# MingXiangL/AttentionShift

Hardware: AMD Instinct MI355X
Metric: images/sec (1024^2, ViT-B) hot path: backbone attention fwd + attention-shift pseudo-labels (higher is better)
Workload: dtype bf16

## Files before the change

attentionshift_amd/_lib.py:

```python
import ctypes
import os

_HERE = os.path.dirname(os.path.abspath(__file__))
LIB_PATH = os.path.join(_HERE, "libattnshift_hip.so")

AS_F32, AS_BF16 = 0, 1

_c_void_p, _c_int, _c_float, _c_size_t = ctypes.c_void_p, ctypes.c_int, ctypes.c_float, ctypes.c_size_t
_c_double = ctypes.c_double

SIGNATURES = {
    "as_version": (_c_int, []),
    "as_last_error": (ctypes.c_char_p, []),
    "as_npad": (_c_int, [_c_int]),
    "as_linear_fwd": (_c_int, [_c_void_p] * 4 + [_c_int] * 5 + [_c_void_p]),
    "as_linear_small_fwd": (_c_int, [_c_void_p, _c_int, _c_void_p, _c_void_p, _c_void_p] + [_c_int] * 5 + [_c_void_p]),
    "as_linear_sk_workspace_bytes": (_c_size_t, [_c_int] * 3),
    "as_linear_sk_fwd": (_c_int, [_c_void_p] * 4 + [_c_int] * 5 + [_c_void_p, _c_size_t, _c_void_p]),
    "as_linear_gelu_fwd": (_c_int, [_c_void_p] * 5 + [_c_int] * 4 + [_c_void_p]),
    "as_linear_dgelu_fwd": (_c_int, [_c_void_p] * 4 + [_c_int] * 4 + [_c_void_p]),
    "as_deconv2x2_fwd": (_c_int, [_c_void_p] * 4 + [_c_int] * 6 + [_c_void_p]),
    "as_qkv_fwd": (_c_int, [_c_void_p] * 6 + [_c_int] * 5 + [_c_void_p]),
    "as_sdpa_fwd_workspace_bytes": (_c_size_t, [_c_int] * 4),
    "as_sdpa_fwd": (_c_int, [_c_void_p] * 6 + [_c_size_t] + [_c_int] * 4 + [_c_void_p]),
# ... 13 lines not shown
    "as_linear_bwd_workspace_bytes": (ctypes.c_size_t, [_c_int] * 3),
    "as_linear_bwd": (_c_int, [_c_void_p] * 6 + [_c_int] * 5 + [_c_void_p, ctypes.c_size_t, _c_void_p]),
    "as_linear_bwd_dgelu": (_c_int, [_c_void_p] * 7 + [_c_int] * 5 + [_c_void_p, ctypes.c_size_t, _c_void_p]),
    "as_assemble_tokens": (_c_int, [_c_void_p] * 3 + [_c_int] * 5 + [_c_void_p]),
    "as_maxpool_nhwc": (_c_int, [_c_void_p] * 2 + [_c_int] * 5 + [ctypes.c_longlong, _c_void_p]),
    "as_mask_count": (_c_int, [_c_void_p] * 2 + [_c_int] * 2 + [_c_void_p]),
    "as_window_attn_bwd_workspace_bytes": (_c_size_t, [_c_int] * 5),
    "as_window_attn_bwd": (_c_int, [_c_void_p] * 8 + [_c_size_t] + [_c_int] * 8 + [_c_void_p]),
    "as_attn_fwd": (_c_int, [_c_void_p] * 12 + [_c_size_t] + [_c_int] * 5 + [_c_void_p]),
    "as_attn_mean_rows": (_c_int, [_c_void_p] * 4 + [_c_int] * 6 + [_c_void_p]),
    "as_rollout_rfrag_bytes": (_c_size_t, [_c_int] * 3),
    "as_rollout_pack": (_c_int, [_c_void_p] * 2 + [_c_int] * 4 + [_c_void_p]),
    "as_rollout_top": (_c_int, [_c_void_p] * 5 + [_c_int] * 5 + [_c_void_p]),
    "as_rollout_step_workspace_bytes": (_c_size_t, [_c_int] * 3),
    "as_rollout_step": (_c_int, [_c_void_p] * 8 + [_c_size_t] + [_c_int] * 5 + [_c_void_p]),
    "as_ccl_2d": (_c_int, [_c_void_p] * 2 + [_c_int] * 3 + [_c_void_p]),
    "as_cam_boxes_workspace_bytes": (_c_size_t, [_c_int] * 4),
    "as_cam_boxes": (_c_int, [_c_void_p] * 2 + [_c_float] * 2 + [_c_int] * 4 + [_c_void_p] * 5 + [_c_size_t, _c_void_p]),
    "as_cam_sample_masks_workspace_bytes": (_c_size_t, [_c_int] * 4),
    "as_cam_sample_masks": (_c_int, [_c_void_p] * 3 + [_c_int] * 4 + [_c_float] * 2 + [_c_void_p] * 3 + [_c_size_t, _c_void_p]),
    "as_mask_candidates_workspace_bytes": (_c_size_t, [_c_int] * 3),
    "as_mask_candidates": (_c_int, [_c_void_p] * 3 + [_c_float] * 3 + [_c_int] + [_c_void_p] * 5 + [_c_size_t]
                           + [_c_int] * 3 + [_c_void_p]),
    "as_part_select": (_c_int, [_c_void_p] * 7 + [_c_int] * 5 + [_c_void_p] * 8 + [_c_void_p]),
    "as_part_stats": (_c_int, [_c_void_p] * 3 + [_c_float] + [_c_void_p] * 4 + [_c_int] * 3 + [_c_void_p]),
    "as_filter_parts": (_c_int, [_c_void_p] * 2 + [_c_float] * 2 + [_c_void_p] + [_c_int] * 3 + [_c_void_p]),
    "as_draw_distinct": (_c_int, [_c_void_p, _c_int, _c_int] + [_c_void_p] * 5 + [_c_int] * 3 + [_c_void_p]),
    "as_mt_sample_ranks": (_c_int, [_c_void_p] * 4 + [_c_int] * 2 + [_c_void_p]),
    "as_mt_perm_ranks": (_c_int, [_c_void_p] * 4 + [_c_int] * 2 + [_c_void_p]),
    "as_small_attn_fwd": (_c_int, [_c_void_p] * 3 + [_c_int] * 5 + [_c_void_p]),
# ... 66 lines not shown
```

attentionshift_amd/csrc/rollout.hip:

```cpp
#include <stdlib.h>
#include "common.h"

namespace {

constexpr int HD = 64, RO_NT = 256;
constexpr float LOG2E = 1.44269504088896340736f;

template <typename T> struct KjCfg { static constexpr int PITCH = HD * (int)sizeof(T) + 16; };

__device__ __forceinline__ size_t rf_slot(int b, int nkb, int i, int k) {
  const int rem = k & 31, s2 = rem >> 4, r16 = rem & 15;
  const int lane = (i & 31) + 32 * ((r16 & 7) >> 2), t = (r16 >> 3) * 4 + (r16 & 3);
  return ((((((size_t)b * nkb + (k >> 5)) * 4 + (i >> 5)) * 2 + s2) * 64) + lane) * 8 + t;
}
__device__ __forceinline__ size_t rf_frag(int b, int nkb, int kb, int ib, int s2, int lane) {
  return ((((((size_t)b * nkb + kb) * 4 + ib) * 2 + s2) * 64) + lane) * 8;
}

template <typename T>
__device__ __forceinline__ f32x16 pbar_tile(const T* __restrict__ q, const T* __restrict__ k,
                                            const float* __restrict__ lse, const char* kj_lds, int b, int h,
                                            int N, int Npad, int i0, int j0, int li, int half) {
  f32x16 pbar;
#pragma unroll
  for (int r = 0; r < 16; ++r) pbar[r] = 0.0f;
  const int irow = min(i0 + li, N - 1);
  const int jrow = min(j0 + li, N - 1);
  for (int hh = 0; hh < h; ++hh) {
    const size_t bh = (size_t)b * h + hh;
    f32x16 s;
#pragma unroll
    for (int r = 0; r < 16; ++r) s[r] = 0.0f;
#pragma unroll
    for (int ks = 0; ks < 4; ++ks) {
      Frag<T> fa, fb;
      fa.load16B(q + qf_frag(bh, Npad, irow, ks, half));
      if (kj_lds != nullptr)
        fb.load16B(reinterpret_cast<const T*>(kj_lds + ((size_t)hh * 32 + li) * KjCfg<T>::PITCH) + ks * 16 + half * 8);
      else
        fb.load16B(k + (bh * Npad + jrow) * HD + ks * 16 + half * 8);
      s = mma32(fa, fb, s);
    }
    const float* lrow = lse + bh * N;
#pragma unroll
    for (int r = 0; r < 16; ++r) {
      const int row = min(i0 + acc_row(r, half), N - 1);
      pbar[r] += __builtin_amdgcn_exp2f(s[r] - lrow[row] * LOG2E);
    }
  }
  const float inv_h = 1.0f / (float)h;
#pragma unroll
  for (int r = 0; r < 16; ++r) pbar[r] *= inv_h;
  return pbar;
}

template <typename T, bool TOP>
__global__ __launch_bounds__(RO_NT) void attn_mean_rows_kernel(const T* __restrict__ q, const T* __restrict__ k,
                                                               const float* __restrict__ lse,
                                                               float* __restrict__ out, T* __restrict__ rf_out, int B,
                                                               int N, int Npad, int h, int row0, int nrows) {
  const int lane = threadIdx.x & 63, wave = threadIdx.x >> 6;
  const int li = lane & 31, half = lane >> 5;
  const int jb = blockIdx.x * 4 + wave, ib = blockIdx.y, b = blockIdx.z;
  const int j0 = jb * 32, i0 = ib * 32;
  if (j0 >= N) return;
  const f32x16 p = pbar_tile<T>(q, k, lse, nullptr, b, h, N, Npad, row0 + i0, j0, li, half);
  const int j = j0 + li;
  const int nkb = (N + 31) / 32;
#pragma unroll
  for (int r = 0; r < 16; ++r) {
    const int i = i0 + acc_row(r, half);
    float v = p[r];
    if (TOP) v = 0.5f * (v + ((row0 + i) == j ? 1.0f : 0.0f));
    const bool live = i < nrows && j < N;
    if (live) out[((size_t)b * nrows + i) * N + j] = v;
    if (rf_out != nullptr && i < 128) rf_out[rf_slot(b, nkb, i, j)] = from_f32<T>(live ? v : 0.0f);
  }
}

template <typename T> struct Kj2 {
  static constexpr int PITCH = sizeof(T) == 2 ? 128 : (HD * 4 + 16);
  __device__ static __forceinline__ int off(int row, int elem) {
    if (sizeof(T) == 2) return row * 128 + ((((elem >> 3) ^ (row & 7))) << 4);
    return row * PITCH + elem * 4;
  }
};

template <typename T, int HPW>
__global__ __launch_bounds__(RO_NT) void rollout_step2_kernel(const T* __restrict__ q, const T* __restrict__ k,
                                                              const float* __restrict__ lse,
                                                              const float* __restrict__ Rin, const T* __restrict__ rf_in,
                                                              float* __restrict__ Rout, T* __restrict__ rf_out,
                                                              float* __restrict__ part, int B, int N, int Npad, int h,
                                                              int Trows, int nsplit, int xbufs) {
  extern __shared__ __attribute__((aligned(16))) char smem[];
  constexpr bool PREFETCH = sizeof(T) == 2;
  const int tid = threadIdx.x, lane = tid & 63, wave = tid >> 6;
  const int li = lane & 31, half = lane >> 5;
  const int j0 = blockIdx.x * 32, b = blockIdx.y, split = blockIdx.z;
  char* kj = smem;
  float4* xchg = reinterpret_cast<float4*>(smem + (size_t)h * 32 * Kj2<T>::PITCH);

  {
    constexpr int CPR = HD * (int)sizeof(T) / 16;
    const int total = h * 32 * CPR;
    for (int c = tid; c < total; c += RO_NT) {
      const int hh = c / (32 * CPR), rem = c % (32 * CPR);
      const int jr = rem / CPR, ch = rem % CPR;
      const int jrow = min(j0 + jr, N - 1);
// ... 97 lines not shown
    if (xbufs == 1) __syncthreads();
  }

  if (own_rows) {
    const int j = j0 + li;
#pragma unroll
    for (int r = 0; r < 16; ++r) {
      const int i = wave * 32 + acc_row(r, half);
      const bool live = i < Trows && j < N;
      if (nsplit > 1) {
        if (live) part[(((size_t)split * B + b) * Trows + i) * N + j] = acc[r];
        continue;
      }
      float v = 0.0f;
      if (live) {
        const size_t idx = ((size_t)b * Trows + i) * N + j;
        v = 0.5f * (acc[r] + Rin[idx]);
        Rout[idx] = v;
      }
      if (rf_out != nullptr) rf_out[rf_slot(b, nkb, i, j)] = from_f32<T>(v);
    }
  }
}

#ifndef AS_ROLLOUT_ABLATE
#define AS_ROLLOUT_ABLATE 0
#endif
template <typename T> __device__ __forceinline__ f32x16 inject_rows(float x, int half);
template <> __device__ __forceinline__ f32x16 inject_rows<float>(float x, int half) {
  f32x16 z;
#pragma unroll
// ... 10 lines not shown
  const __bf16 mid = (__bf16)r1;
  const __bf16 lo = (__bf16)(r1 - (float)mid);
  const __bf16 zero = (__bf16)0.0f, one = (__bf16)1.0f;
  Frag<__bf16> fa, fb;
  fa.v = bf16x8{hi, mid, lo, zero, zero, zero, zero, zero};
  fb.v = bf16x8{one, one, one, zero, zero, zero, zero, zero};
  return mma32(fa, fb, z);
}

template <typename T>
__global__ __launch_bounds__(RO_NT, 3) void rollout_step3_kernel(const T* __restrict__ q, const T* __restrict__ k,
                                                                 const float* __restrict__ lse,
                                                                 const float* __restrict__ Rin, const T* __restrict__ rf_in,
                                                                 float* __restrict__ Rout, T* __restrict__ rf_out,
                                                                 float* __restrict__ part, int B, int N, int Npad, int h,
                                                                 int Trows, int nsplit) {
  extern __shared__ __attribute__((aligned(16))) char smem[];
  const int tid = threadIdx.x, lane = tid & 63, wave = tid >> 6;
  const int li = lane & 31, half = lane >> 5;
  const int j0 = blockIdx.x * 32, b = blockIdx.y, split = blockIdx.z;
  char* kj = smem;
  {
    constexpr int CPR = HD * (int)sizeof(T) / 16;
    const int total = h * 32 * CPR;
    for (int c = tid; c < total; c += RO_NT) {
      const int hh = c / (32 * CPR), rem = c % (32 * CPR);
      const int jr = rem / CPR, ch = rem % CPR;
      const int jrow = min(j0 + jr, N - 1);
      const uint4 u = *reinterpret_cast<const uint4*>(
          reinterpret_cast<const char*>(k + (((size_t)b * h + hh) * Npad + jrow) * HD) + ch * 16);
      const int elem = ch * (16 / (int)sizeof(T));
// ... 92 lines not shown
                   red[((2 * 2 + x) * 16 + r) * 64 + lane]) + red[((3 * 2 + x) * 16 + r) * 64 + lane];
    }
  }
  if (wave * 32 < Trows) {
    const int j = j0 + li;
#pragma unroll
    for (int r = 0; r < 16; ++r) {
      const int i = wave * 32 + acc_row(r, half);
      const bool live = i < Trows && j < N;
      if (nsplit > 1) {
        if (live) part[(((size_t)split * B + b) * Trows + i) * N + j] = mine[r];
        continue;
      }
      float v = 0.0f;
      if (live) {
        const size_t idx = ((size_t)b * Trows + i) * N + j;
        v = 0.5f * (mine[r] + Rin[idx]);
        Rout[idx] = v;
      }
      if (rf_out != nullptr) rf_out[rf_slot(b, nkb, i, j)] = from_f32<T>(v);
    }
  }
}

constexpr int R4_HPG = 4;
constexpr int R4_QBYTES = R4_HPG * 4 * 1024;
constexpr int R4_LSE = R4_QBYTES + 8 * 1024;
constexpr int R4_STAGE = R4_LSE + 1024;
#ifndef AS_R4_OCC1
#define AS_R4_OCC1 3
#endif
template <int NIB> struct R4Cfg { static constexpr int NSTAGE = NIB == 1 ? 2 : 3, OCC = NIB == 1 ? AS_R4_OCC1 : 2; };

typedef __attribute__((ext_vector_type(4))) unsigned r4_u32x4;
template <int OFF> __device__ __forceinline__ void r4_lds_read128(r4_u32x4& dst, unsigned addr) {
  asm volatile("ds_read_b128 %0, %1 offset:%2" : "=v"(dst) : "v"(addr), "n"(OFF));
}
__device__ __forceinline__ void r4_lds_read128_dyn(r4_u32x4& dst, unsigned addr) {
  asm volatile("ds_read_b128 %0, %1" : "=v"(dst) : "v"(addr));
}
__device__ __forceinline__ void r4_wait_lds(r4_u32x4& a, r4_u32x4& b, r4_u32x4& c, r4_u32x4& d) {
  asm volatile("s_waitcnt lgkmcnt(0)" : "+v"(a), "+v"(b), "+v"(c), "+v"(d));
  __builtin_amdgcn_sched_barrier(0);
}
__device__ __forceinline__ void r4_wait_lds8(r4_u32x4& a, r4_u32x4& b, r4_u32x4& c, r4_u32x4& d, r4_u32x4& e, r4_u32x4& f,
                                             r4_u32x4& g, r4_u32x4& h) {
  asm volatile("s_waitcnt lgkmcnt(0)" : "+v"(a), "+v"(b), "+v"(c), "+v"(d), "+v"(e), "+v"(f), "+v"(g), "+v"(h));
// ... 10 lines not shown
__device__ __forceinline__ void r4_dma16(unsigned voff, const char* sbase, unsigned dst) {
  unsigned keep;
  asm volatile("s_mov_b32 %0, m0\n\ts_mov_b32 m0, %3\n\ts_nop 0\n\tglobal_load_lds_dwordx4 %1, %2\n\ts_mov_b32 m0, %0"
               : "=&s"(keep) : "v"(voff), "s"(sbase), "s"(dst) : "memory");
}
__device__ __forceinline__ void r4_dma4(unsigned voff, const char* sbase, unsigned dst) {
  unsigned keep;
  asm volatile("s_mov_b32 %0, m0\n\ts_mov_b32 m0, %3\n\ts_nop 0\n\tglobal_load_lds_dword %1, %2\n\ts_mov_b32 m0, %0"
               : "=&s"(keep) : "v"(voff), "s"(sbase), "s"(dst) : "memory");
}

template <int NIB>
__global__ __launch_bounds__(RO_NT, R4Cfg<NIB>::OCC) void rollout_step4_kernel(const __bf16* __restrict__ q, const __bf16* __restrict__ k,
                                                                 const float* __restrict__ lse, const __bf16* __restrict__ rf_in,
                                                                 float* __restrict__ part, int B, int N, int Npad, int h,
                                                                 int Trows, int ksplit) {
  extern __shared__ __attribute__((aligned(16))) char smem[];
  constexpr int R4_NSTAGE = R4Cfg<NIB>::NSTAGE;
  const int tid = threadIdx.x, lane = tid & 63, wave = __builtin_amdgcn_readfirstlane(tid >> 6);
  const int li = lane & 31, half = lane >> 5;
  const int ngroups = h / R4_HPG;
  const int j0 = blockIdx.x * 128 + wave * 32, b = blockIdx.y;
  const int hg = blockIdx.z % ngroups, split = blockIdx.z / ngroups;
  const int nkb = (N + 31) / 32;
  const int nib = min((Trows + 31) / 32, NIB);
  const int kb0 = (int)((long long)nkb * split / ksplit), kb1 = (int)((long long)nkb * (split + 1) / ksplit);
  const int nblk = kb1 - kb0;
  const size_t bh0 = (size_t)b * h + hg * R4_HPG;

  Frag<__bf16> fk[R4_HPG][4];
  {
// ... 28 lines not shown
#pragma unroll
    for (int r = 0; r < 16; ++r) acc[ib][r] = 0.0f;
  const float inv_h = 1.0f / (float)h;
  const unsigned lbase = (unsigned)(size_t)(const __attribute__((address_space(3))) char*)smem + lane * 16;

  if (nblk > 0) stage(kb0, 0);
  if (R4_NSTAGE > 2 && nblk > 1) stage(kb0 + 1, 1);

  for (int it = 0; it < nblk; ++it) {
    const int kb = kb0 + it, buf = it % R4_NSTAGE;
    if (AS_ROLLOUT_ABLATE != 11) {
      if (R4_NSTAGE == 2 || it + 1 >= nblk) asm volatile("s_waitcnt vmcnt(0)" ::: "memory");
      else if (NIB == 4 || wave == 0) asm volatile("s_waitcnt vmcnt(7)" ::: "memory");
      else asm volatile("s_waitcnt vmcnt(5)" ::: "memory");
    }
    {
      float own;
      const unsigned a_own = (unsigned)(size_t)(const __attribute__((address_space(3))) char*)smem + buf * R4_STAGE + R4_LSE + wave * 256 + lane * 4;
      asm volatile("ds_read_b32 %0, %1\n\ts_waitcnt lgkmcnt(0)" : "=v"(own) : "v"(a_own) : "memory");
      own *= -LOG2E;
      asm volatile("ds_write_b32 %0, %1\n\ts_waitcnt lgkmcnt(0)" :: "v"(a_own), "v"(own) : "memory");
    }
    if (AS_ROLLOUT_ABLATE != 14) __builtin_amdgcn_s_barrier();
    if (AS_ROLLOUT_ABLATE != 11 && it + R4_NSTAGE - 1 < nblk) stage(kb + R4_NSTAGE - 1, (it + R4_NSTAGE - 1) % R4_NSTAGE);
    const unsigned sb = lbase + buf * R4_STAGE;
    const unsigned cb = (unsigned)(size_t)(const __attribute__((address_space(3))) char*)smem + buf * R4_STAGE + R4_LSE + half * 16;
    r4_u32x4 fc[2][4];
    auto read_c = [&](int hh, r4_u32x4 (&c)[4]) {
      const unsigned a = cb + hh * 256;
      r4_lds_read128_dyn(c[0], a);
      r4_lds_read128<32>(c[1], a);
// ... 79 lines not shown
    __builtin_amdgcn_sched_barrier(0);
#pragma unroll
    for (int s2 = 0; s2 < 2; ++s2)
#pragma unroll
      for (int ib = 0; ib < NIB; ++ib)
        if (ib < nib) {
          Frag<__bf16> f;
          f.v = *reinterpret_cast<bf16x8*>(&fr[ib][s2]);
          if (AS_ROLLOUT_ABLATE != 15) acc[ib] = mma32(f, fp[s2], acc[ib]);
          else acc[ib][0] += (float)f.v[0] + (float)fp[s2].v[0];
        }
  }

  const int pidx = split * ngroups + hg;
  const int j = j0 + li;
  if (j < N) {
#pragma unroll
    for (int ib = 0; ib < NIB; ++ib)
#pragma unroll
      for (int r = 0; r < 16; ++r) {
        const int i = ib * 32 + acc_row(r, half);
        if (i < Trows) part[(((size_t)pidx * B + b) * Trows + i) * N + j] = acc[ib][r] * inv_h;
      }
  }
}

bool rollout_force_v3() {
  static const bool v = getenv("AS_ROLLOUT_V3") != nullptr;
  return v;
}

constexpr int R4_MAXPARTS = 16;
int rollout4_ksplit(int B, int N, int h, int slots) {
  static const int forced = [] { const char* e = getenv("AS_R4_KS"); return e ? atoi(e) : 0; }();
  if (forced > 0 && forced * (h / R4_HPG) <= 16) return forced;
  const int units = as_ceil_div(N, 128) * B * (h / R4_HPG);
  int best = 1;
  float best_eff = 0.0f;
  for (int ks = 1; ks * (h / R4_HPG) <= R4_MAXPARTS && ks <= 8; ++ks) {
    const int wgs = units * ks;
    const float eff = (float)wgs / (float)(as_ceil_div(wgs, slots) * slots);
    if (eff > best_eff + 0.02f) { best_eff = eff; best = ks; }
  }
  return best;
}

template <typename T>
__global__ __launch_bounds__(64) void rollout_finish_kernel(const float* __restrict__ part, const float* __restrict__ Rin,
                                                            float* __restrict__ Rout, T* __restrict__ rf_out, int B, int N,
                                                            int Trows, int nsplit) {
  const int nkb = (N + 31) / 32;
  const int j = blockIdx.x * 64 + threadIdx.x, i = blockIdx.y, b = blockIdx.z;
  if (j >= nkb * 32) return;
  float v = 0.0f;
  if (i < Trows && j < N) {
    const size_t idx = ((size_t)b * Trows + i) * N + j;
    float a = 0.0f;
    for (int sp = 0; sp < nsplit; ++sp) a += part[(size_t)sp * B * Trows * N + idx];
    v = 0.5f * (a + Rin[idx]);
    Rout[idx] = v;
  }
  if (rf_out != nullptr) rf_out[rf_slot(b, nkb, i, j)] = from_f32<T>(v);
}

template <typename T>
int launch_rollout_step2(const void* q, const void* k, const float* lse, const float* Rin, const void* rf_in, float* Rout,
                         void* rf_out, float* part, int nsplit, int B, int N, int h, int Trows, hipStream_t s) {
  const int Npad = as_round_up(N, 64);
  const int hpw = as_ceil_div(h, 4);
  dim3 grid(as_ceil_div(N, 32), B, nsplit);
  const size_t kbytes = (size_t)h * 32 * Kj2<T>::PITCH, slab = 4 * 4 * 64 * sizeof(float4);
  const int xbufs = kbytes + 2 * slab <= 160 * 1024 ? 2 : 1;
  const size_t lds = kbytes + xbufs * slab;
  AS_REQUIRE(lds <= 160 * 1024, AS_E_UNSUPPORTED, "rollout_step: LDS %zu B exceeds 160 KiB (h=%d)", lds, h);
#define AS_RO2(HPW)                                                                                            \
  do {                                                                                                         \
    (void)hipFuncSetAttribute((const void*)rollout_step2_kernel<T, HPW>, hipFuncAttributeMaxDynamicSharedMemorySize, \
                              (int)lds);                                                                       \
    hipLaunchKernelGGL((rollout_step2_kernel<T, HPW>), grid, dim3(RO_NT), lds, s, (const T*)q, (const T*)k, lse, Rin, \
                       (const T*)rf_in, Rout, (T*)rf_out, part, B, N, Npad, h, Trows, nsplit, xbufs);          \
  } while (0)
  if (sizeof(T) == 2 && h % R4_HPG == 0 && part != nullptr && nsplit == R4_MAXPARTS && !rollout_force_v3()) {
    const int ng = h / R4_HPG;
    const int ks = rollout4_ksplit(B, N, h, 512);
    const size_t lds4 = (size_t)(Trows <= 32 ? R4Cfg<1>::NSTAGE : R4Cfg<4>::NSTAGE) * R4_STAGE;
    if (Trows <= 32) {
      (void)hipFuncSetAttribute((const void*)rollout_step4_kernel<1>, hipFuncAttributeMaxDynamicSharedMemorySize, (int)lds4);
      hipLaunchKernelGGL(rollout_step4_kernel<1>, dim3(as_ceil_div(N, 128), B, ks * ng), dim3(RO_NT), lds4, s, (const __bf16*)q,
                         (const __bf16*)k, lse, (const __bf16*)rf_in, part, B, N, Npad, h, Trows, ks);
    } else {
      (void)hipFuncSetAttribute((const void*)rollout_step4_kernel<4>, hipFuncAttributeMaxDynamicSharedMemorySize, (int)lds4);
      hipLaunchKernelGGL(rollout_step4_kernel<4>, dim3(as_ceil_div(N, 128), B, ks * ng), dim3(RO_NT), lds4, s, (const __bf16*)q,
                         (const __bf16*)k, lse, (const __bf16*)rf_in, part, B, N, Npad, h, Trows, ks);
    }
    AS_CHECK_LAUNCH("rollout_step4");
    dim3 fg(as_ceil_div(as_ceil_div(N, 32) * 32, 64), as_round_up(Trows, 32), B);
    hipLaunchKernelGGL((rollout_finish_kernel<T>), fg, dim3(64), 0, s, (const float*)part, Rin, Rout, (T*)rf_out, B, N,
                       Trows, ks * ng);
    AS_CHECK_LAUNCH("rollout_finish");
    return AS_OK;
  }
  if (sizeof(T) == 2 && h >= 8 && (getenv("AS_ROLLOUT_V2") == nullptr)) {
    const size_t lds3 = (size_t)h * 32 * Kj2<T>::PITCH;
    (void)hipFuncSetAttribute((const void*)rollout_step3_kernel<T>, hipFuncAttributeMaxDynamicSharedMemorySize, (int)lds3);
    hipLaunchKernelGGL((rollout_step3_kernel<T>), grid, dim3(RO_NT), lds3, s, (const T*)q, (const T*)k, lse, Rin,
                       (const T*)rf_in, Rout, (T*)rf_out, part, B, N, Npad, h, Trows, nsplit);
  } else {
  switch (hpw) {
    case 1: AS_RO2(1); break;
    case 2: AS_RO2(2); break;
    case 3: AS_RO2(3); break;
    case 4: AS_RO2(4); break;
    default: AS_REQUIRE(false, AS_E_UNSUPPORTED, "rollout_step: h=%d heads (max 16)", h);
  }
  }
#undef AS_RO2
  AS_CHECK_LAUNCH("rollout_step2");
  if (nsplit > 1) {
    dim3 fg(as_ceil_div(as_ceil_div(N, 32) * 32, 64), as_round_up(Trows, 32), B);
    hipLaunchKernelGGL((rollout_finish_kernel<T>), fg, dim3(64), 0, s, (const float*)part, Rin, Rout, (T*)rf_out, B, N,
                       Trows, nsplit);
    AS_CHECK_LAUNCH("rollout_finish");
  }
  return AS_OK;
}

int rollout_nsplit(int B, int N) {
  const int wgs = as_ceil_div(N, 32) * B;
  int ns = 1;
  while (ns < 16 && wgs * ns < 2048) ns *= 2;
  return wgs >= 2048 ? 1 : ns;
}

template <typename T>
int launch_mean_rows(const void* q, const void* k, const float* lse, float* out, void* rf_out, int B, int N, int h,
                     int row0, int nrows, bool top, hipStream_t s) {
  const int Npad = as_round_up(N, 64);
  dim3 grid(as_ceil_div(as_ceil_div(N, 32), 4), as_ceil_div(nrows, 32), B);
  if (top)
    hipLaunchKernelGGL((attn_mean_rows_kernel<T, true>), grid, dim3(RO_NT), 0, s, (const T*)q, (const T*)k, lse,
                       out, (T*)rf_out, B, N, Npad, h, row0, nrows);
  else
    hipLaunchKernelGGL((attn_mean_rows_kernel<T, false>), grid, dim3(RO_NT), 0, s, (const T*)q, (const T*)k, lse,
                       out, (T*)rf_out, B, N, Npad, h, row0, nrows);
  AS_CHECK_LAUNCH("attn_mean_rows");
  return AS_OK;
}

}

extern "C" size_t as_rollout_rfrag_bytes(int B, int N, int dtype) {
  if (B <= 0 || N <= 0) return 0;
  return (size_t)B * as_ceil_div(N, 32) * 4 * 2 * 64 * 8 * (dtype == AS_BF16 ? 2 : 4);
}

extern "C" int as_attn_mean_rows(const void* q, const void* k, const float* lse, float* out, int B, int N, int h,
                                 int row0, int nrows, int dtype, as_stream_t stream) {
  AS_REQUIRE(q && k && lse && out, AS_E_BADARG, "as_attn_mean_rows: null pointer");
  AS_REQUIRE(B > 0 && N > 0 && h > 0 && row0 >= 0 && nrows > 0 && row0 + nrows <= N, AS_E_BADARG,
// ... 27 lines not shown

extern "C" int as_rollout_pack(const float* R, void* rf, int B, int N, int T, int dtype, as_stream_t stream) {
  AS_REQUIRE(R && rf, AS_E_BADARG, "as_rollout_pack: null pointer");
  AS_REQUIRE(B > 0 && N > 0 && T > 0 && T <= 128, AS_E_BADARG, "as_rollout_pack: bad sizes N=%d T=%d", N, T);
  dim3 grid(as_ceil_div(as_ceil_div(N, 32) * 32, 64), as_round_up(T, 32), B);
  if (dtype == AS_BF16)
    hipLaunchKernelGGL(rollout_pack_kernel<__bf16>, grid, dim3(64), 0, (hipStream_t)stream, R, (__bf16*)rf, B, N, T);
  else if (dtype == AS_F32)
    hipLaunchKernelGGL(rollout_pack_kernel<float>, grid, dim3(64), 0, (hipStream_t)stream, R, (float*)rf, B, N, T);
  else
    AS_REQUIRE(false, AS_E_UNSUPPORTED, "as_rollout_pack: dtype %d", dtype);
  AS_CHECK_LAUNCH("rollout_pack");
  return AS_OK;
}

extern "C" size_t as_rollout_step_workspace_bytes(int B, int N, int T) {
  if (B <= 0 || N <= 0 || T <= 0) return 0;
  return (size_t)R4_MAXPARTS * B * T * N * sizeof(float);
}

extern "C" int as_rollout_step(const void* q, const void* k, const float* lse, const float* R_in, const void* rf_in,
                               float* R_out, void* rf_out, void* workspace, size_t workspace_bytes, int B, int N, int h,
                               int T, int dtype, as_stream_t stream) {
  AS_REQUIRE(q && k && lse && R_in && rf_in && R_out && R_in != R_out && rf_in != rf_out, AS_E_BADARG,
             "as_rollout_step: null/aliased pointer");
  AS_REQUIRE(B > 0 && h > 0 && h <= 16 && T > 0 && T <= N && T <= 128, AS_E_BADARG,
             "as_rollout_step: bad sizes N=%d T=%d h=%d", N, T, h);
  hipStream_t s = (hipStream_t)stream;
  const size_t need = as_rollout_step_workspace_bytes(B, N, T);
  const bool have_ws = workspace != nullptr && workspace_bytes >= need && need > 0;
  const bool stream4 = have_ws && dtype == AS_BF16 && h % R4_HPG == 0 && !rollout_force_v3();
  const int ns = stream4 ? R4_MAXPARTS : (have_ws ? rollout_nsplit(B, N) : 1);
  float* part = ns > 1 ? (float*)workspace : nullptr;
  if (dtype == AS_BF16)
    return launch_rollout_step2<__bf16>(q, k, lse, R_in, rf_in, R_out, rf_out, part, ns, B, N, h, T, s);
  if (dtype == AS_F32) return launch_rollout_step2<float>(q, k, lse, R_in, rf_in, R_out, rf_out, part, ns, B, N, h, T, s);
  AS_REQUIRE(false, AS_E_UNSUPPORTED, "as_rollout_step: dtype %d", dtype);
}
```

attentionshift_amd/ops.py:

```python
import ctypes
import os

import threading

import numpy as np
import torch

from . import _lib
from ._lib import AS_BF16, AS_F32, AttnShiftError

HEAD_DIM = 64


def _dt(t):
    if t.dtype == torch.float32:
        return AS_F32
    if t.dtype == torch.bfloat16:
        return AS_BF16
    raise AttnShiftError(f"unsupported dtype {t.dtype} (float32 or bfloat16)")


def _chk(*tensors, dtype=None):
    for t in tensors:
        if t is None:
# ... 453 lines not shown


def attn_mean_rows(state, row0, nrows):
    lib = _lib.load()
    out = torch.empty(state.B, nrows, state.N, device=state.q.device, dtype=torch.float32)
    _lib.check(lib.as_attn_mean_rows(_p(state.q), _p(state.k), _p(state.lse), _p(out), state.B, state.N, state.h,
                                     int(row0), int(nrows), _dt(state.q), _stream()), "as_attn_mean_rows")
    return out


def rollout_rows(states, num_point_tokens, rows=None, use_workspace=True):
    lib = _lib.load()
    top = states[-1]
    T = int(num_point_tokens)
    dev, dt = top.q.device, _dt(top.q)
    nbytes = lib.as_rollout_rfrag_bytes(top.B, top.N, dt)
    outs = []
    R = torch.empty(top.B, T, top.N, device=dev, dtype=torch.float32)
    lower = list(reversed(states[:-1]))
    subset = rows is not None and len(lower) > 0
    rf = torch.empty(nbytes, device=dev, dtype=torch.uint8) if not subset else None
    _lib.check(lib.as_rollout_top(_p(top.q), _p(top.k), _p(top.lse), _p(R), _p(rf), top.B, top.N, top.h, T, dt, _stream()),
               "as_rollout_top")
    if rows is not None:
        R = torch.gather(R, 1, rows[:, :, None].expand(-1, -1, top.N)).contiguous()
        T = R.shape[1]
        if subset:
            rf = torch.empty(nbytes, device=dev, dtype=torch.uint8)
            _lib.check(lib.as_rollout_pack(_p(R), _p(rf), top.B, top.N, T, dt, _stream()), "as_rollout_pack")
    outs.append(R)
# ... 533 lines not shown
```

include/attnshift.h:

```cpp
#ifndef ATTNSHIFT_H
#define ATTNSHIFT_H

#include <stddef.h>
#include <stdint.h>

#ifdef __cplusplus
extern "C" {
#endif

#define AS_VERSION 100
#define AS_OK 0
#define AS_E_BADARG (-1)
#define AS_E_UNSUPPORTED (-2)
#define AS_E_LAUNCH (-3)
#define AS_E_WORKSPACE (-4)

#define AS_F32 0
#define AS_BF16 1

#define AS_HEAD_DIM 64

typedef void* as_stream_t;

int as_version(void);
// ... 81 lines not shown
int as_window_attn_bwd(const void* qkv, const float* bqkv, const float* table, const void* d_out, void* dqkv,
                       float* dtable, float* dbqkv_pad, void* workspace, size_t workspace_bytes, int B, int H, int W,
                       int C, int h, int ws, int shift, int dtype, as_stream_t stream);

int as_attn_mean_rows(const void* q, const void* k, const float* lse, float* out, int B, int N, int h,
                      int row0, int nrows, int dtype, as_stream_t stream);

size_t as_rollout_rfrag_bytes(int B, int N, int dtype);
int as_rollout_pack(const float* R, void* rf, int B, int N, int T, int dtype, as_stream_t stream);
size_t as_rollout_step_workspace_bytes(int B, int N, int T);
int as_rollout_top(const void* q, const void* k, const float* lse, float* R_out, void* rf_out, int B, int N, int h,
                   int T, int dtype, as_stream_t stream);
int as_rollout_step(const void* q, const void* k, const float* lse, const float* R_in, const void* rf_in,
                    float* R_out, void* rf_out, void* workspace, size_t workspace_bytes, int B, int N, int h, int T,
                    int dtype, as_stream_t stream);


int as_ccl_2d(const uint8_t* img , int32_t* labels , int M, int H, int W,
              as_stream_t stream);

size_t as_cam_boxes_workspace_bytes(int M, int Hp, int Wp, int up);
int as_cam_boxes(const float* cams , const float* points , float cam_thr,
                 float area_ratio, int M, int Hp, int Wp, int up, float* boxes, int32_t* status,
                 float* cams_up, float* minmax, void* ws, size_t ws_bytes, as_stream_t stream);

size_t as_cam_sample_masks_workspace_bytes(int G, int Hp, int Wp, int up);
int as_cam_sample_masks(const float* cams , const int32_t* map_idx ,
                        const float* minmax , int G, int Hp, int Wp, int up, float thr_bg, float thr_fg,
                        uint8_t* masks, int32_t* counts, void* ws, size_t ws_bytes, as_stream_t stream);

// ... 110 lines not shown
```

Before: 328.6.

## Fuse attention rollout chain into one host call with in-kernel split-K finish

Adds as_rollout_chain, which runs the whole multi-layer attention rollout in one C call with a single workspace. The top layer's row gather moves into the mean-rows kernel via a rowsel index, and outputs go into one strided buffer, which removes the Python loop, per-layer allocations, torch.gather and pack calls. For small row counts, the split-K step4 kernel now reduces its partials itself: the last-arriving block, found with an atomic ticket counter, does the sum, so the separate finish kernel launch is dropped. pbar_tile also batches several heads' fragment and LSE loads before the MMAs to improve latency hiding, at the cost of more registers.

Result: slower. 323.8 (-1.5%).

```diff
diff --git a/attentionshift_amd/_lib.py b/attentionshift_amd/_lib.py
--- a/attentionshift_amd/_lib.py
+++ b/attentionshift_amd/_lib.py
@@ -51,6 +51,9 @@
     "as_rollout_top": (_c_int, [_c_void_p] * 5 + [_c_int] * 5 + [_c_void_p]),
     "as_rollout_step_workspace_bytes": (_c_size_t, [_c_int] * 3),
     "as_rollout_step": (_c_int, [_c_void_p] * 8 + [_c_size_t] + [_c_int] * 5 + [_c_void_p]),
+    "as_rollout_chain_workspace_bytes": (_c_size_t, [_c_int] * 5),
+    "as_rollout_chain": (_c_int, [_c_void_p] * 3 + [_c_int, _c_void_p, _c_int] + [_c_void_p] * 2 + [_c_size_t] + [_c_int] * 5
+                         + [_c_void_p]),
     "as_ccl_2d": (_c_int, [_c_void_p] * 2 + [_c_int] * 3 + [_c_void_p]),
     "as_cam_boxes_workspace_bytes": (_c_size_t, [_c_int] * 4),
     "as_cam_boxes": (_c_int, [_c_void_p] * 2 + [_c_float] * 2 + [_c_int] * 4 + [_c_void_p] * 5 + [_c_size_t, _c_void_p]),
diff --git a/attentionshift_amd/csrc/rollout.hip b/attentionshift_amd/csrc/rollout.hip
--- a/attentionshift_amd/csrc/rollout.hip
+++ b/attentionshift_amd/csrc/rollout.hip
@@ -17,35 +17,49 @@
   return ((((((size_t)b * nkb + kb) * 4 + ib) * 2 + s2) * 64) + lane) * 8;
 }
 
-template <typename T>
+template <typename T, typename RowOf>
 __device__ __forceinline__ f32x16 pbar_tile(const T* __restrict__ q, const T* __restrict__ k,
                                             const float* __restrict__ lse, const char* kj_lds, int b, int h,
-                                            int N, int Npad, int i0, int j0, int li, int half) {
+                                            int N, int Npad, RowOf row_of, int j0, int li, int half) {
   f32x16 pbar;
 #pragma unroll
   for (int r = 0; r < 16; ++r) pbar[r] = 0.0f;
-  const int irow = min(i0 + li, N - 1);
+  const int irow = row_of(li);
   const int jrow = min(j0 + li, N - 1);
-  for (int hh = 0; hh < h; ++hh) {
-    const size_t bh = (size_t)b * h + hh;
-    f32x16 s;
-#pragma unroll
-    for (int r = 0; r < 16; ++r) s[r] = 0.0f;
-#pragma unroll
-    for (int ks = 0; ks < 4; ++ks) {
-      Frag<T> fa, fb;
-      fa.load16B(q + qf_frag(bh, Npad, irow, ks, half));
-      if (kj_lds != nullptr)
-        fb.load16B(reinterpret_cast<const T*>(kj_lds + ((size_t)hh * 32 + li) * KjCfg<T>::PITCH) + ks * 16 + half * 8);
-      else
-        fb.load16B(k + (bh * Npad + jrow) * HD + ks * 16 + half * 8);
-      s = mma32(fa, fb, s);
-    }
-    const float* lrow = lse + bh * N;
-#pragma unroll
-    for (int r = 0; r < 16; ++r) {
-      const int row = min(i0 + acc_row(r, half), N - 1);
-      pbar[r] += __builtin_amdgcn_exp2f(s[r] - lrow[row] * LOG2E);
+  int arow[16];
+#pragma unroll
+  for (int r = 0; r < 16; ++r) arow[r] = row_of(acc_row(r, half));
+  constexpr int HU = sizeof(T) == 2 ? 4 : 2;
+  for (int h0 = 0; h0 < h; h0 += HU) {
+    Frag<T> fa[HU][4], fb[HU][4];
+    float lv[HU][16];
+#pragma unroll
+    for (int u = 0; u < HU; ++u) {
+      const int hh = min(h0 + u, h - 1);
+      const size_t bh = (size_t)b * h + hh;
+#pragma unroll
+      for (int ks = 0; ks < 4; ++ks) {
+        fa[u][ks].load16B(q + qf_frag(bh, Npad, irow, ks, half));
+        if (kj_lds != nullptr)
+          fb[u][ks].load16B(reinterpret_cast<const T*>(kj_lds + ((size_t)hh * 32 + li) * KjCfg<T>::PITCH) + ks * 16 + half * 8);
+        else
+          fb[u][ks].load16B(k + (bh * Npad + jrow) * HD + ks * 16 + half * 8);
+      }
+      const float* lrow = lse + bh * N;
+#pragma unroll
+      for (int r = 0; r < 16; ++r) lv[u][r] = lrow[arow[r]];
+    }
+#pragma unroll
+    for (int u = 0; u < HU; ++u) {
+      if (h0 + u >= h) break;
+      f32x16 s;
+#pragma unroll
+      for (int r = 0; r < 16; ++r) s[r] = 0.0f;
+#pragma unroll
+      for (int ks = 0; ks < 4; ++ks) s = mma32(fa[u][ks], fb[u][ks], s);
+#pragma unroll
+      for (int r = 0; r < 16; ++r)
+        pbar[r] += __builtin_amdgcn_exp2f(s[r] - lv[u][r] * LOG2E);
     }
   }
   const float inv_h = 1.0f / (float)h;
@@ -58,22 +72,28 @@
 __global__ __launch_bounds__(RO_NT) void attn_mean_rows_kernel(const T* __restrict__ q, const T* __restrict__ k,
                                                                const float* __restrict__ lse,
                                                                float* __restrict__ out, T* __restrict__ rf_out, int B,
-                                                               int N, int Npad, int h, int row0, int nrows) {
+                                                               int N, int Npad, int h, int row0, int nrows,
+                                                               const long long* __restrict__ rowsel, size_t ostride) {
   const int lane = threadIdx.x & 63, wave = threadIdx.x >> 6;
   const int li = lane & 31, half = lane >> 5;
   const int jb = blockIdx.x * 4 + wave, ib = blockIdx.y, b = blockIdx.z;
   const int j0 = jb * 32, i0 = ib * 32;
   if (j0 >= N) return;
-  const f32x16 p = pbar_tile<T>(q, k, lse, nullptr, b, h, N, Npad, row0 + i0, j0, li, half);
+  auto row_of = [&](int x) {
+    if (rowsel == nullptr) return min(row0 + i0 + x, N - 1);
+    const long long s = rowsel[(size_t)b * nrows + min(i0 + x, nrows - 1)];
+    return row0 + (int)min(max(s, 0ll), (long long)(N - 1 - row0));
+  };
+  const f32x16 p = pbar_tile<T>(q, k, lse, nullptr, b, h, N, Npad, row_of, j0, li, half);
   const int j = j0 + li;
   const int nkb = (N + 31) / 32;
 #pragma unroll
   for (int r = 0; r < 16; ++r) {
     const int i = i0 + acc_row(r, half);
     float v = p[r];
-    if (TOP) v = 0.5f * (v + ((row0 + i) == j ? 1.0f : 0.0f));
+    if (TOP) v = 0.5f * (v + (row_of(acc_row(r, half)) == j ? 1.0f : 0.0f));
     const bool live = i < nrows && j < N;
-    if (live) out[((size_t)b * nrows + i) * N + j] = v;
+    if (live) out[(size_t)b * ostride + (size_t)i * N + j] = v;
     if (rf_out != nullptr && i < 128) rf_out[rf_slot(b, nkb, i, j)] = from_f32<T>(live ? v : 0.0f);
   }
 }
@@ -92,7 +112,7 @@
                                                               const float* __restrict__ Rin, const T* __restrict__ rf_in,
                                                               float* __restrict__ Rout, T* __restrict__ rf_out,
                                                               float* __restrict__ part, int B, int N, int Npad, int h,
-                                                              int Trows, int nsplit, int xbufs) {
+                                                              int Trows, int nsplit, int xbufs, size_t rstride) {
   extern __shared__ __attribute__((aligned(16))) char smem[];
   constexpr bool PREFETCH = sizeof(T) == 2;
   const int tid = threadIdx.x, lane = tid & 63, wave = tid >> 6;
@@ -220,7 +240,7 @@
       }
       float v = 0.0f;
       if (live) {
-        const size_t idx = ((size_t)b * Trows + i) * N + j;
+        const size_t idx = (size_t)b * rstride + (size_t)i * N + j;
         v = 0.5f * (acc[r] + Rin[idx]);
         Rout[idx] = v;
       }
@@ -261,7 +281,7 @@
                                                                  const float* __restrict__ Rin, const T* __restrict__ rf_in,
                                                                  float* __restrict__ Rout, T* __restrict__ rf_out,
                                                                  float* __restrict__ part, int B, int N, int Npad, int h,
-                                                                 int Trows, int nsplit) {
+                                                                 int Trows, int nsplit, size_t rstride) {
   extern __shared__ __attribute__((aligned(16))) char smem[];
   const int tid = threadIdx.x, lane = tid & 63, wave = tid >> 6;
   const int li = lane & 31, half = lane >> 5;
@@ -384,7 +404,7 @@
       }
       float v = 0.0f;
       if (live) {
-        const size_t idx = ((size_t)b * Trows + i) * N + j;
+        const size_t idx = (size_t)b * rstride + (size_t)i * N + j;
         v = 0.5f * (mine[r] + Rin[idx]);
         Rout[idx] = v;
       }
@@ -401,6 +421,14 @@
 #define AS_R4_OCC1 3
 #endif
 template <int NIB> struct R4Cfg { static constexpr int NSTAGE = NIB == 1 ? 2 : 3, OCC = NIB == 1 ? AS_R4_OCC1 : 2; };
+constexpr int R4_MAXPARTS = 16;
+struct R4Finish {
+  unsigned* cnt;
+  const float* Rin;
+  float* Rout;
+  __bf16* rf_out;
+  size_t rstride;
+};
 
 typedef __attribute__((ext_vector_type(4))) unsigned r4_u32x4;
 template <int OFF> __device__ __forceinline__ void r4_lds_read128(r4_u32x4& dst, unsigned addr) {
@@ -441,7 +469,7 @@
 __global__ __launch_bounds__(RO_NT, R4Cfg<NIB>::OCC) void rollout_step4_kernel(const __bf16* __restrict__ q, const __bf16* __restrict__ k,
                                                                  const float* __restrict__ lse, const __bf16* __restrict__ rf_in,
                                                                  float* __restrict__ part, int B, int N, int Npad, int h,
-                                                                 int Trows, int ksplit) {
+                                                                 int Trows, int ksplit, R4Finish fin) {
   extern __shared__ __attribute__((aligned(16))) char smem[];
   constexpr int R4_NSTAGE = R4Cfg<NIB>::NSTAGE;
   const int tid = threadIdx.x, lane = tid & 63, wave = __builtin_amdgcn_readfirstlane(tid >> 6);
@@ -500,7 +528,7 @@
       else if (NIB == 4 || wave == 0) asm volatile("s_waitcnt vmcnt(7)" ::: "memory");
       else asm volatile("s_waitcnt vmcnt(5)" ::: "memory");
     }
-    {
+    if (AS_ROLLOUT_ABLATE != 16) {
       float own;
       const unsigned a_own = (unsigned)(size_t)(const __attribute__((address_space(3))) char*)smem + buf * R4_STAGE + R4_LSE + wave * 256 + lane * 4;
       asm volatile("ds_read_b32 %0, %1\n\ts_waitcnt lgkmcnt(0)" : "=v"(own) : "v"(a_own) : "memory");
@@ -610,14 +638,71 @@
 
   const int pidx = split * ngroups + hg;
   const int j = j0 + li;
+  const bool fused = fin.cnt != nullptr;
   if (j < N) {
 #pragma unroll
     for (int ib = 0; ib < NIB; ++ib)
 #pragma unroll
       for (int r = 0; r < 16; ++r) {
         const int i = ib * 32 + acc_row(r, half);
-        if (i < Trows) part[(((size_t)pidx * B + b) * Trows + i) * N + j] = acc[ib][r] * inv_h;
-      }
+        float* dst = part + (((size_t)pidx * B + b) * Trows + i) * N + j;
+        const float v = acc[ib][r] * inv_h;
+        if (i < Trows) {
+          if (fused) __hip_atomic_store(dst, v, __ATOMIC_RELAXED, __HIP_MEMORY_SCOPE_AGENT);
+          else *dst = v;
+        }
+      }
+  }
+  if (!fused) return;
+
+  asm volatile("s_waitcnt vmcnt(0)" ::: "memory");
+  __syncthreads();
+  unsigned* last_flag = reinterpret_cast<unsigned*>(smem);
+  const int nparts = ksplit * ngroups;
+  const int tf = wave * 64 + li + 32 * half;
+  if (tf == 0) {
+    unsigned* c = fin.cnt + (size_t)b * gridDim.x + blockIdx.x;
+    const unsigned ticket = __hip_atomic_fetch_add(c, 1u, __ATOMIC_RELAXED, __HIP_MEMORY_SCOPE_AGENT);
+    const bool last = ticket == (unsigned)(nparts - 1);
+    if (last) __hip_atomic_store(c, 0u, __ATOMIC_RELAXED, __HIP_MEMORY_SCOPE_AGENT);
+    *last_flag = last ? 1u : 0u;
+  }
+  __syncthreads();
+  if (__builtin_amdgcn_readfirstlane((int)*last_flag) == 0) return;
+  const int jf = blockIdx.x * 128 + (tf & 127);
+  if (jf >= nkb * 32) return;
+  const size_t pstride = (size_t)B * Trows * N;
+  for (int i0 = tf >> 7; i0 < nib * 32; i0 += 4) {
+    float v[2] = {0.0f, 0.0f};
+    if (i0 < Trows && jf < N) {
+      const int i1 = min(i0 + 2, Trows - 1);
+      const float* p0 = part + ((size_t)b * Trows + i0) * N + jf;
+      const float* p1 = part + ((size_t)b * Trows + i1) * N + jf;
+      float pv[2][R4_MAXPARTS], a[2] = {0.0f, 0.0f};
+#pragma unroll
+      for (int sp = 0; sp < R4_MAXPARTS; ++sp) {
+        const size_t o = (size_t)min(sp, nparts - 1) * pstride;
+        pv[0][sp] = __hip_atomic_load(p0 + o, __ATOMIC_RELAXED, __HIP_MEMORY_SCOPE_AGENT);
+        pv[1][sp] = __hip_atomic_load(p1 + o, __ATOMIC_RELAXED, __HIP_MEMORY_SCOPE_AGENT);
+      }
+      const size_t idx0 = (size_t)b * fin.rstride + (size_t)i0 * N + jf, idx1 = (size_t)b * fin.rstride + (size_t)i1 * N + jf;
+      const float r0 = fin.Rin[idx0], r1 = fin.Rin[idx1];
+#pragma unroll
+      for (int sp = 0; sp < R4_MAXPARTS; ++sp) {
+        a[0] = sp < nparts ? a[0] + pv[0][sp] : a[0];
+        a[1] = sp < nparts ? a[1] + pv[1][sp] : a[1];
+      }
+      v[0] = 0.5f * (a[0] + r0);
+      fin.Rout[idx0] = v[0];
+      if (i0 + 2 < Trows) {
+        v[1] = 0.5f * (a[1] + r1);
+        fin.Rout[idx1] = v[1];
+      }
+    }
+    if (fin.rf_out != nullptr) {
+      fin.rf_out[rf_slot(b, nkb, i0, jf)] = from_f32<__bf16>(v[0]);
+      fin.rf_out[rf_slot(b, nkb, i0 + 2, jf)] = from_f32<__bf16>(v[1]);
+    }
   }
 }
 
@@ -626,7 +711,6 @@
   return v;
 }
 
-constexpr int R4_MAXPARTS = 16;
 int rollout4_ksplit(int B, int N, int h, int slots) {
   static const int forced = [] { const char* e = getenv("AS_R4_KS"); return e ? atoi(e) : 0; }();
   if (forced > 0 && forced * (h / R4_HPG) <= 16) return forced;
@@ -644,15 +728,16 @@
 template <typename T>
 __global__ __launch_bounds__(64) void rollout_finish_kernel(const float* __restrict__ part, const float* __restrict__ Rin,
                                                             float* __restrict__ Rout, T* __restrict__ rf_out, int B, int N,
-                                                            int Trows, int nsplit) {
+                                                            int Trows, int nsplit, size_t rstride) {
   const int nkb = (N + 31) / 32;
   const int j = blockIdx.x * 64 + threadIdx.x, i = blockIdx.y, b = blockIdx.z;
   if (j >= nkb * 32) return;
   float v = 0.0f;
   if (i < Trows && j < N) {
-    const size_t idx = ((size_t)b * Trows + i) * N + j;
+    const size_t pidx = ((size_t)b * Trows + i) * N + j;
+    const size_t idx = (size_t)b * rstride + (size_t)i * N + j;
     float a = 0.0f;
-    for (int sp = 0; sp < nsplit; ++sp) a += part[(size_t)sp * B * Trows * N + idx];
+    for (int sp = 0; sp < nsplit; ++sp) a += part[(size_t)sp * B * Trows * N + pidx];
     v = 0.5f * (a + Rin[idx]);
     Rout[idx] = v;
   }
@@ -661,7 +746,8 @@
 
 template <typename T>
 int launch_rollout_step2(const void* q, const void* k, const float* lse, const float* Rin, const void* rf_in, float* Rout,
-                         void* rf_out, float* part, int nsplit, int B, int N, int h, int Trows, hipStream_t s) {
+                         void* rf_out, float* part, int nsplit, int B, int N, int h, int Trows, hipStream_t s,
+                         size_t rstride, unsigned* cnt = nullptr) {
   const int Npad = as_round_up(N, 64);
   const int hpw = as_ceil_div(h, 4);
   dim3 grid(as_ceil_div(N, 32), B, nsplit);
@@ -674,25 +760,28 @@
     (void)hipFuncSetAttribute((const void*)rollout_step2_kernel<T, HPW>, hipFuncAttributeMaxDynamicSharedMemorySize, \
                               (int)lds);                                                                       \
     hipLaunchKernelGGL((rollout_step2_kernel<T, HPW>), grid, dim3(RO_NT), lds, s, (const T*)q, (const T*)k, lse, Rin, \
-                       (const T*)rf_in, Rout, (T*)rf_out, part, B, N, Npad, h, Trows, nsplit, xbufs);          \
+                       (const T*)rf_in, Rout, (T*)rf_out, part, B, N, Npad, h, Trows, nsplit, xbufs, rstride); \
   } while (0)
   if (sizeof(T) == 2 && h % R4_HPG == 0 && part != nullptr && nsplit == R4_MAXPARTS && !rollout_force_v3()) {
     const int ng = h / R4_HPG;
     const int ks = rollout4_ksplit(B, N, h, 512);
     const size_t lds4 = (size_t)(Trows <= 32 ? R4Cfg<1>::NSTAGE : R4Cfg<4>::NSTAGE) * R4_STAGE;
+    R4Finish fin = {nullptr, Rin, Rout, (__bf16*)rf_out, rstride};
     if (Trows <= 32) {
+      fin.cnt = cnt;
       (void)hipFuncSetAttribute((const void*)rollout_step4_kernel<1>, hipFuncAttributeMaxDynamicSharedMemorySize, (int)lds4);
       hipLaunchKernelGGL(rollout_step4_kernel<1>, dim3(as_ceil_div(N, 128), B, ks * ng), dim3(RO_NT), lds4, s, (const __bf16*)q,
-                         (const __bf16*)k, lse, (const __bf16*)rf_in, part, B, N, Npad, h, Trows, ks);
+                         (const __bf16*)k, lse, (const __bf16*)rf_in, part, B, N, Npad, h, Trows, ks, fin);
     } else {
       (void)hipFuncSetAttribute((const void*)rollout_step4_kernel<4>, hipFuncAttributeMaxDynamicSharedMemorySize, (int)lds4);
       hipLaunchKernelGGL(rollout_step4_kernel<4>, dim3(as_ceil_div(N, 128), B, ks * ng), dim3(RO_NT), lds4, s, (const __bf16*)q,
-                         (const __bf16*)k, lse, (const __bf16*)rf_in, part, B, N, Npad, h, Trows, ks);
+                         (const __bf16*)k, lse, (const __bf16*)rf_in, part, B, N, Npad, h, Trows, ks, fin);
     }
     AS_CHECK_LAUNCH("rollout_step4");
+    if (fin.cnt != nullptr) return AS_OK;
     dim3 fg(as_ceil_div(as_ceil_div(N, 32) * 32, 64), as_round_up(Trows, 32), B);
     hipLaunchKernelGGL((rollout_finish_kernel<T>), fg, dim3(64), 0, s, (const float*)part, Rin, Rout, (T*)rf_out, B, N,
-                       Trows, ks * ng);
+                       Trows, ks * ng, rstride);
     AS_CHECK_LAUNCH("rollout_finish");
     return AS_OK;
   }
@@ -700,7 +789,7 @@
     const size_t lds3 = (size_t)h * 32 * Kj2<T>::PITCH;
     (void)hipFuncSetAttribute((const void*)rollout_step3_kernel<T>, hipFuncAttributeMaxDynamicSharedMemorySize, (int)lds3);
     hipLaunchKernelGGL((rollout_step3_kernel<T>), grid, dim3(RO_NT), lds3, s, (const T*)q, (const T*)k, lse, Rin,
-                       (const T*)rf_in, Rout, (T*)rf_out, part, B, N, Npad, h, Trows, nsplit);
+                       (const T*)rf_in, Rout, (T*)rf_out, part, B, N, Npad, h, Trows, nsplit, rstride);
   } else {
   switch (hpw) {
     case 1: AS_RO2(1); break;
@@ -715,7 +804,7 @@
   if (nsplit > 1) {
     dim3 fg(as_ceil_div(as_ceil_div(N, 32) * 32, 64), as_round_up(Trows, 32), B);
     hipLaunchKernelGGL((rollout_finish_kernel<T>), fg, dim3(64), 0, s, (const float*)part, Rin, Rout, (T*)rf_out, B, N,
-                       Trows, nsplit);
+                       Trows, nsplit, rstride);
     AS_CHECK_LAUNCH("rollout_finish");
   }
   return AS_OK;
@@ -730,15 +819,16 @@
 
 template <typename T>
 int launch_mean_rows(const void* q, const void* k, const float* lse, float* out, void* rf_out, int B, int N, int h,
-                     int row0, int nrows, bool top, hipStream_t s) {
+                     int row0, int nrows, bool top, hipStream_t s, const long long* rowsel = nullptr, size_t ostride = 0) {
+  if (ostride == 0) ostride = (size_t)nrows * N;
   const int Npad = as_round_up(N, 64);
   dim3 grid(as_ceil_div(as_ceil_div(N, 32), 4), as_ceil_div(nrows, 32), B);
   if (top)
     hipLaunchKernelGGL((attn_mean_rows_kernel<T, true>), grid, dim3(RO_NT), 0, s, (const T*)q, (const T*)k, lse,
-                       out, (T*)rf_out, B, N, Npad, h, row0, nrows);
+                       out, (T*)rf_out, B, N, Npad, h, row0, nrows, rowsel, ostride);
   else
     hipLaunchKernelGGL((attn_mean_rows_kernel<T, false>), grid, dim3(RO_NT), 0, s, (const T*)q, (const T*)k, lse,
-                       out, (T*)rf_out, B, N, Npad, h, row0, nrows);
+                       out, (T*)rf_out, B, N, Npad, h, row0, nrows, rowsel, ostride);
   AS_CHECK_LAUNCH("attn_mean_rows");
   return AS_OK;
 }
@@ -796,6 +886,22 @@
   return AS_OK;
 }
 
+namespace {
+int rollout_step_any(const void* q, const void* k, const float* lse, const float* R_in, const void* rf_in, float* R_out,
+                     void* rf_out, void* workspace, int B, int N, int h, int T, int dtype, hipStream_t s, size_t rstride,
+                     unsigned* cnt) {
+  const bool have_ws = workspace != nullptr;
+  const bool stream4 = have_ws && dtype == AS_BF16 && h % R4_HPG == 0 && !rollout_force_v3();
+  const int ns = stream4 ? R4_MAXPARTS : (have_ws ? rollout_nsplit(B, N) : 1);
+  float* part = ns > 1 ? (float*)workspace : nullptr;
+  if (dtype == AS_BF16)
+    return launch_rollout_step2<__bf16>(q, k, lse, R_in, rf_in, R_out, rf_out, part, ns, B, N, h, T, s, rstride, cnt);
+  if (dtype == AS_F32)
+    return launch_rollout_step2<float>(q, k, lse, R_in, rf_in, R_out, rf_out, part, ns, B, N, h, T, s, rstride, cnt);
+  AS_REQUIRE(false, AS_E_UNSUPPORTED, "as_rollout_step: dtype %d", dtype);
+}
+}
+
 extern "C" size_t as_rollout_step_workspace_bytes(int B, int N, int T) {
   if (B <= 0 || N <= 0 || T <= 0) return 0;
   return (size_t)R4_MAXPARTS * B * T * N * sizeof(float);
@@ -808,14 +914,65 @@
              "as_rollout_step: null/aliased pointer");
   AS_REQUIRE(B > 0 && h > 0 && h <= 16 && T > 0 && T <= N && T <= 128, AS_E_BADARG,
              "as_rollout_step: bad sizes N=%d T=%d h=%d", N, T, h);
-  hipStream_t s = (hipStream_t)stream;
   const size_t need = as_rollout_step_workspace_bytes(B, N, T);
   const bool have_ws = workspace != nullptr && workspace_bytes >= need && need > 0;
-  const bool stream4 = have_ws && dtype == AS_BF16 && h % R4_HPG == 0 && !rollout_force_v3();
-  const int ns = stream4 ? R4_MAXPARTS : (have_ws ? rollout_nsplit(B, N) : 1);
-  float* part = ns > 1 ? (float*)workspace : nullptr;
+  return rollout_step_any(q, k, lse, R_in, rf_in, R_out, rf_out, have_ws ? workspace : nullptr, B, N, h, T, dtype,
+                          (hipStream_t)stream, (size_t)T * N, nullptr);
+}
+
+namespace {
+struct ChainLayout { size_t cnt, part, rf, total; };
+ChainLayout rollout_chain_layout(int B, int N, int Lc, int Trows, int dtype) {
+  ChainLayout w = {0, 0, 0, 0};
+  if (B <= 0 || N <= 0 || Lc <= 1 || Trows <= 0) return w;
+  auto up256 = [](size_t x) { return (x + 255) / 256 * 256; };
+  w.cnt = up256((size_t)(Lc - 1) * B * as_ceil_div(N, 128) * sizeof(unsigned));
+  w.part = up256(as_rollout_step_workspace_bytes(B, N, Trows));
+  w.rf = up256(as_rollout_rfrag_bytes(B, N, dtype));
+  w.total = w.cnt + w.part + 2 * w.rf;
+  return w;
+}
+}
+
+extern "C" size_t as_rollout_chain_workspace_bytes(int B, int N, int Lc, int Trows, int dtype) {
+  return rollout_chain_layout(B, N, Lc, Trows, dtype).total;
+}
+
+extern "C" int as_rollout_chain(const void* const* q, const void* const* k, const float* const* lse, int Lc,
+                                const int64_t* rows, int G, float* out, void* workspace, size_t workspace_bytes, int B,
+                                int N, int h, int T, int dtype, as_stream_t stream) {
+  AS_REQUIRE(q && k && lse && out && Lc > 0, AS_E_BADARG, "as_rollout_chain: null pointer");
+  for (int l = 0; l < Lc; ++l) AS_REQUIRE(q[l] && k[l] && lse[l], AS_E_BADARG, "as_rollout_chain: null pointer (layer %d)", l);
+  AS_REQUIRE(B > 0 && h > 0 && h <= 16 && T > 0 && T <= N && T <= 128 && (rows == nullptr || (G > 0 && G <= 128)), AS_E_BADARG,
+             "as_rollout_chain: bad sizes N=%d T=%d h=%d G=%d", N, T, h, G);
+  AS_REQUIRE(dtype == AS_BF16 || dtype == AS_F32, AS_E_UNSUPPORTED, "as_rollout_chain: dtype %d", dtype);
+  hipStream_t s = (hipStream_t)stream;
+  const int Trows = rows != nullptr ? G : T;
+  const ChainLayout w = rollout_chain_layout(B, N, Lc, Trows, dtype);
+  AS_REQUIRE(w.total == 0 || (workspace != nullptr && workspace_bytes >= w.total), AS_E_BADARG,
+             "as_rollout_chain: workspace %zu B < %zu B", workspace_bytes, w.total);
+  const size_t rstride = (size_t)Lc * Trows * N;
+  char* ws = (char*)workspace;
+  unsigned* cnt = (unsigned*)ws;
+  void* part = ws + w.cnt;
+  void* rf[2] = {ws + w.cnt + w.part, ws + w.cnt + w.part + w.rf};
+  const bool fused = Lc > 1 && dtype == AS_BF16 && h % R4_HPG == 0 && !rollout_force_v3() && Trows <= 32;
+  if (fused) AS_REQUIRE(hipMemsetAsync(cnt, 0, w.cnt, s) == hipSuccess, AS_E_LAUNCH, "as_rollout_chain: counter memset failed");
+  const int top = Lc - 1;
+  int rc;
   if (dtype == AS_BF16)
-    return launch_rollout_step2<__bf16>(q, k, lse, R_in, rf_in, R_out, rf_out, part, ns, B, N, h, T, s);
-  if (dtype == AS_F32) return launch_rollout_step2<float>(q, k, lse, R_in, rf_in, R_out, rf_out, part, ns, B, N, h, T, s);
-  AS_REQUIRE(false, AS_E_UNSUPPORTED, "as_rollout_step: dtype %d", dtype);
-}
+    rc = launch_mean_rows<__bf16>(q[top], k[top], lse[top], out, Lc > 1 ? rf[0] : nullptr, B, N, h, N - T, Trows, true, s,
+                                  (const long long*)rows, rstride);
+  else
+    rc = launch_mean_rows<float>(q[top], k[top], lse[top], out, Lc > 1 ? rf[0] : nullptr, B, N, h, N - T, Trows, true, s,
+                                 (const long long*)rows, rstride);
+  if (rc != AS_OK) return rc;
+  for (int n = 1; n < Lc; ++n) {
+    const int l = top - n;
+    rc = rollout_step_any(q[l], k[l], lse[l], out + (size_t)(n - 1) * Trows * N, rf[(n - 1) & 1], out + (size_t)n * Trows * N,
+                          n + 1 < Lc ? rf[n & 1] : nullptr, part, B, N, h, Trows, dtype, s, rstride,
+                          fused ? cnt + (size_t)(n - 1) * B * as_ceil_div(N, 128) : nullptr);
+    if (rc != AS_OK) return rc;
+  }
+  return AS_OK;
+}
diff --git a/attentionshift_amd/ops.py b/attentionshift_amd/ops.py
--- a/attentionshift_amd/ops.py
+++ b/attentionshift_amd/ops.py
@@ -491,6 +491,19 @@
     top = states[-1]
     T = int(num_point_tokens)
     dev, dt = top.q.device, _dt(top.q)
+    if use_workspace:
+        Lc = len(states)
+        G = 0 if rows is None else int(rows.shape[1])
+        Trows = T if rows is None else G
+        if rows is not None:
+            rows = rows.to(device=dev, dtype=torch.int64).contiguous()
+        out = torch.empty(top.B, Lc, Trows, top.N, device=dev, dtype=torch.float32)
+        wbytes = lib.as_rollout_chain_workspace_bytes(top.B, top.N, Lc, Trows, dt)
+        ws = torch.empty(wbytes, device=dev, dtype=torch.uint8) if wbytes else None
+        ptrs = [(ctypes.c_void_p * Lc)(*[_p(getattr(st, f)) for st in states]) for f in ("q", "k", "lse")]
+        _lib.check(lib.as_rollout_chain(ptrs[0], ptrs[1], ptrs[2], Lc, _p(rows), G, _p(out), _p(ws), wbytes, top.B, top.N,
+                                        top.h, T, dt, _stream()), "as_rollout_chain")
+        return out
     nbytes = lib.as_rollout_rfrag_bytes(top.B, top.N, dt)
     outs = []
     R = torch.empty(top.B, T, top.N, device=dev, dtype=torch.float32)
diff --git a/include/attnshift.h b/include/attnshift.h
--- a/include/attnshift.h
+++ b/include/attnshift.h
@@ -119,6 +119,10 @@
 int as_rollout_step(const void* q, const void* k, const float* lse, const float* R_in, const void* rf_in,
                     float* R_out, void* rf_out, void* workspace, size_t workspace_bytes, int B, int N, int h, int T,
                     int dtype, as_stream_t stream);
+size_t as_rollout_chain_workspace_bytes(int B, int N, int Lc, int Trows, int dtype);
+int as_rollout_chain(const void* const* q, const void* const* k, const float* const* lse, int Lc, const int64_t* rows,
+                     int G, float* out, void* workspace, size_t workspace_bytes, int B, int N, int h, int T, int dtype,
+                     as_stream_t stream);
 
 
 int as_ccl_2d(const uint8_t* img , int32_t* labels , int M, int H, int W,
```
